# ymxlzgy/echoscene

Measured on AMD Instinct MI355X. Metric: denoising steps/sec (layout+SDF) for 32-node scene-graph, 64^3 SDF (3x16^3 latent), full step = one DDPM layout step + one DDIM shape step over all objects; `value` = the FUSED step (both loops as one hipGraph per step, the layout step on a parallel branch: what the K timed steps ran); `full_steps_p, higher is better.
Workload: dtype f16 MFMA operands / f32 accumulate (shape UNet); f32 (layout, GCN)

## Files before the change

echoscene_amd/csrc/es_vol.hip:

```cpp
#include "es_common.h"
#include <string>
#include <algorithm>
#include <cstdlib>
#include <initializer_list>
#include <utility>
#include <type_traits>

namespace {

__device__ __forceinline__ int f_swz(int row) { return (0x1320 >> (((row >> 2) & 3) * 4)) & 3; }

constexpr int GN_VT = 64;

__global__ __launch_bounds__(256) void k_gn_partial(const es_gn_args a, float* part, int vt) {
    __shared__ float ssum4[4][2048], ssq4[4][2048];
    float* ssum = ssum4[0];
    float* ssq = ssq4[0];
    const int o = blockIdx.y, tile = blockIdx.x, C = a.C1 + a.C2;
    const int v0 = tile * vt;
    const int nv = min(vt, a.V - v0);
    const int c4n = C >> 2;
    const int CX = 64;
    const int cx = threadIdx.x & (CX - 1), vy = threadIdx.x >> 6;
    for (int c4 = cx; c4 < c4n; c4 += CX) {
// ... 390 lines not shown
        const int w = (gy - p * Pw) < Pw ? (gy - p * Pw) : Pw;
        bx = rr / w;
        by = p * Pw + (rr - bx * w);
    } else {
        bx = t % gx;
        by = t / gx;
    }
}

__device__ __forceinline__ void* uniform_ptr(const void* p) {
    const unsigned long v = (unsigned long)p;
    const unsigned lo = (unsigned)__builtin_amdgcn_readfirstlane((int)(unsigned)v), hi = (unsigned)__builtin_amdgcn_readfirstlane((int)(unsigned)(v >> 32));
    return (void*)(((unsigned long)hi << 32) | lo);
}

template <int BM_, int NW_, bool ACTIVE = true, bool LOWREG = false, int EPI_ = -1, bool NOSYNC = false, bool STATS_ = false, bool FOLD_ = false>
__device__ __forceinline__ void conv_epilogue(const es_conv_args& a, const ConvGeom& g, f4 (&acc)[BM_ / (NW_ / 2) / 16][7],
                                              char* smem, long M, long m0, int n0, int wave, int lane, int S, int bz,
                                              int ncdhw) {
    constexpr int WROWS = BM_ / (NW_ / 2), MI = WROWS / 16;
    const bool geglu_epi = EPI_ < 0 ? a.epilogue == ES_EPI_GEGLU : EPI_ == ES_EPI_GEGLU;
    if constexpr (!ACTIVE) {
        __syncthreads();
        return;
    }
    const int wm = wave >> 1, wn = wave & 1, i16 = lane & 15, q = lane >> 4;
    const int V = g.D * g.H * g.W;
    if constexpr (!NOSYNC) __syncthreads();
    float* slab = (float*)smem + wave * (16 * 116);
    const bool vec_ok = !ncdhw && (a.N % 4 == 0) && (a.out_ld % 4 == 0) && (!a.rowvec || a.rowvec_ld % 4 == 0);
    float* part = S > 1 ? (float*)a.workspace + (long)bz * M * a.N : nullptr;
    if (geglu_epi) {
        const bool lo = i16 < 8;
        const int cw = i16 & 7;
#pragma unroll
        for (int j = 0; j < 7; ++j) {
            const float bj = a.bias[n0 + wn * 112 + j * 16 + i16];
#pragma unroll
            for (int i = 0; i < MI; ++i)
#pragma unroll
                for (int r = 0; r < 4; ++r) acc[i][j][r] += bj;
        }
        constexpr int HLD = 72;
        _Float16* hslab = (_Float16*)smem + wave * (16 * HLD);
        typedef unsigned int u4g __attribute__((ext_vector_type(4)));
        const int rr = q * 4 + (lo ? 0 : 2);
// ... 120 lines not shown
                }
                return;
            }
            f4 rbuf[2][8];
            write_slab(0);
            __builtin_amdgcn_sched_barrier(0);
            load_res_s(0, rbuf[0]);
            __builtin_amdgcn_sched_barrier(0);
#pragma unroll
            for (int i = 0; i < MI; ++i) {
                __builtin_amdgcn_s_waitcnt(0xc07f);
                __builtin_amdgcn_wave_barrier();
                if (i >= 1 && i + 1 < MI) load_res_s(i + 1, rbuf[(i + 1) & 1]);
                __builtin_amdgcn_sched_barrier(0);
                combine_s(i, rbuf[i & 1]);
                __builtin_amdgcn_sched_barrier(0);
                __builtin_amdgcn_wave_barrier();
                if (i + 1 < MI) write_slab(i + 1);
                __builtin_amdgcn_sched_barrier(0);
                if (i == 0 && MI > 1) load_res_s(1, rbuf[1]);
                __builtin_amdgcn_sched_barrier(0);
            }
            if constexpr (STATS_) {
                static_assert(WROWS == 64, "row groups of gn_stats_out are 64 rows");
                f4 os, oq;
#pragma unroll
                for (int e = 0; e < 4; ++e) { os[e] = __shfl(gs[e], lane + 28); oq[e] = __shfl(gq[e], lane + 28); }
                if (lane < 28 && n_ok && rows_left > 0) {
                    const unsigned nrg = (unsigned)((M + 63) >> 6);
                    const unsigned so = (unsigned)(mw0 >> 6) * (unsigned)a.N + (unsigned)n;
                    *(f4*)&a.gn_stats_out[so] = gs + os;
                    *(f4*)&a.gn_stats_out[so + nrg * (unsigned)a.N] = gq + oq;
                }
            }
        }
        return;
    }
#pragma unroll
    for (int i = 0; i < MI; ++i) {
        if (vec_ok) {
#pragma unroll
            for (int j = 0; j < 7; ++j)
#pragma unroll
                for (int r = 0; r < 4; ++r) slab[(q * 4 + r) * 116 + j * 16 + i16] = acc[i][j][r];
            __builtin_amdgcn_s_waitcnt(0xc07f);
            __builtin_amdgcn_wave_barrier();
            {
                typedef unsigned int u4e __attribute__((ext_vector_type(4)));
                typedef unsigned int u2e __attribute__((ext_vector_type(2)));
                constexpr unsigned OOBE = 0x80000000u;
                const long rb = m0 + wm * WROWS + i * 16;
                const int vshe = g.lw + g.lh + g.ld;
                float* const o32 = part ? part + rb * a.N : (a.out_f32 ? a.out_f32 + rb * a.out_ld : nullptr);
                const unsigned ldp = part ? (unsigned)a.N : (unsigned)a.out_ld, lde = (unsigned)a.out_ld;
                const bool ep = !part;
// ... 592 lines not shown
    conv_tile_of(a, bx, by, bz);
    const int S = gridDim.z;
    int ks_begin, ks_end;
    split_range(a.taps * (a.Cin >> 5), a.a2 ? (a.Cin2 >> 5) : 0, a.taps, bz, S, ks_begin, ks_end);
    conv_ws_tile<BM_, NC_, NP_, UP_, EPI_, STATS_, NS_>(a, g, ncdhw, smem, wave, lane, M, bx, by, ks_begin, ks_end, S, bz, stamp);
}

template <bool STATS_>
__global__ __launch_bounds__(768, 3) void k_conv_ws_fold(const es_conv_args a, const ConvGeom g) {
    extern __shared__ __attribute__((aligned(16))) char smem[];
    const int tid = threadIdx.x, lane = tid & 63;
    const int wave = __builtin_amdgcn_readfirstlane(tid >> 6);
    unsigned long long* stamp = nullptr;
#ifdef ES_STAMP
    stamp = g_stamp_buf ? g_stamp_buf + ((size_t)(blockIdx.x + gridDim.x * (blockIdx.y + gridDim.y * blockIdx.z)) * 12 + wave) * 8 : nullptr;
#endif
    ES_STAMP_AT(0);
    const long M = (long)g.O * g.D * g.H * g.W;
    int bx, by, bz;
    conv_tile_of(a, bx, by, bz);
    conv_ws_tile<256, 8, 4, true, ES_EPI_NONE, STATS_, 3, true>(a, g, 0, smem, wave, lane, M, bx, by, 0, 12 * (a.Cin >> 5), 1, 0, stamp);
}

typedef int i4v __attribute__((ext_vector_type(4)));
template <int DIR>
__device__ __forceinline__ h8 a3_shift(const h8 v, const bool zero_lane) {
    i4v x = __builtin_bit_cast(i4v, v);
#pragma unroll
    for (int e = 0; e < 4; ++e) {
        const int s = DIR < 0 ? __builtin_amdgcn_update_dpp(0, x[e], 0x111, 0xf, 0xf, true) : __builtin_amdgcn_update_dpp(0, x[e], 0x101, 0xf, 0xf, true);
        x[e] = zero_lane ? 0 : s;
    }
    return __builtin_bit_cast(h8, x);
}

template <bool STATS_>
__global__ __launch_bounds__(768, 3) void k_conv_ws3(const es_conv_args a, const ConvGeom g) {
    constexpr int BM_ = 256, NC_ = 8, NP_ = 4, NSB = 7, MI = 4;
    constexpr int A_BYTES = BM_ * BK * 2, B_BYTES = BNP * BK * 2, A_RING = NSB * B_BYTES;
    constexpr int NA = (BM_ / 16) / NP_, NB = (BNP / 16) / NP_;
    constexpr unsigned OOB = 0x80000000u;
    typedef __attribute__((address_space(3))) void* lds_ptr;
    extern __shared__ __attribute__((aligned(16))) char smem[];
    const int tid = threadIdx.x, lane = tid & 63;
    const int wave = __builtin_amdgcn_readfirstlane(tid >> 6);
    const long M = (long)g.O * g.D * g.H * g.W;
// ... 1277 lines not shown
    "ws_256_up_fold", "linear_ws", "linear_deep", "lean_256", "lean_128", "lean_64"
};
static_assert(sizeof(kConvKernelName) / sizeof(kConvKernelName[0]) == (size_t)ConvKernel::lean_64 + 1, "kConvKernelName: one name per ConvKernel value");
enum class ConvReduce { none, plain, gn_part };
struct ConvRoute {
    ConvGeom g;
    int ncdhw;
    long M;
    long omax;
    ConvKernel kernel;
    dim3 grid;
    size_t lds;
    int S;
    int ncb;
    bool upm, geglu;
    char unbuilt[96];
    bool epi_stats;
    bool stats;
    bool part_ok;
    ConvReduce reduce;
    int vt;
    bool stats_pass;
    int slabs;
};
}

constexpr int LDS256 = 3 * (256 * BK * 2 + BNP * BK * 2), LDS128 = 3 * (128 * BK * 2 + BNP * BK * 2), LDS64 = 3 * (64 * BK * 2 + BNP * BK * 2);
constexpr int LDSLIN = LDS256 + 8 * 16 * 116 * 4;
constexpr int LDSDEEP = 7 * (64 * BK * 2 + BNP * BK * 2);
constexpr int LDSWS3 = 9 * 16384;

static int conv_route(const es_conv_args* a, ConvRoute* r) {
    *r = ConvRoute{};
    ES_REQUIRE(a->Cin % 32 == 0 && a->Cin > 0, "es_conv_mfma_f16: Cin=%d must be a positive multiple of 32", a->Cin);
    ES_REQUIRE(a->taps == 27 || a->taps == 1, "es_conv_mfma_f16: taps=%d", a->taps);
    ES_REQUIRE(!a->a2 || (a->Cin2 % 32 == 0 && a->Cin2 > 0), "es_conv_mfma_f16: Cin2=%d", a->Cin2);
    ES_REQUIRE(a->out_f32 || a->out_f16, "es_conv_mfma_f16: no output");
    ES_REQUIRE(a->epilogue == ES_EPI_NONE || (a->epilogue == ES_EPI_GEGLU && a->N % 224 == 0 && a->out_f16 && !a->out_f32 && !a->res &&
                                              !a->rowvec && !a->a2 && a->bias && a->out_ld >= a->N / 2 && a->out_ld % 8 == 0 && a->splitk <= 1),
               "es_conv_mfma_f16: GEGLU epilogue needs N %% 224 == 0 (N=%d), bias, f16 output only, no split-K", a->N);
    ConvGeom& g = r->g;
    g.O = a->O; g.D = a->D; g.H = a->H; g.W = a->W;
    g.Hi = a->H; g.Wi = a->W;
    g.Di = a->D;
    if (a->mode == ES_CONV_DOWN_HW) { g.Hi = 2 * a->H; g.Wi = 2 * a->W; }
    ES_REQUIRE(a->mode >= ES_CONV_SAME && a->mode <= ES_CONV_DOWN_DHW_P01, "es_conv_mfma_f16: unknown mode %d", a->mode);
// ... 179 lines not shown
    } else if (st_bm) {
        const int np = vo("conv_st_np"), ns = vo("conv_st_ns");
        if (st_bm == 64 && np == 4 && ns == 3) r->kernel = ConvKernel::ws_64_4_4_3;
        else if (st_bm == 64 && np == 4 && ns == 6) r->kernel = ConvKernel::ws_64_4_4_6;
        else if (st_bm == 128 && np == 4 && ns == 3) r->kernel = ConvKernel::ws_128_4_4_3;
        else if (st_bm == 128 && np == 8 && ns == 3) r->kernel = ConvKernel::ws_128_4_8_3;
        else if (st_bm == 128 && np == 8 && ns == 5) r->kernel = ConvKernel::ws_128_4_8_5;
        else snprintf(r->unbuilt, sizeof(r->unbuilt), "conv_st_bm=%d conv_st_np=%d conv_st_ns=%d is not a built tile", st_bm, np, ns);
        r->grid = dim3((unsigned)((M + st_bm - 1) / st_bm), uy, S);
    } else if (deep) {
        S = 1;
        r->kernel = ConvKernel::linear_deep;
        r->grid = dim3((unsigned)((M + 63) / 64), uy, 1);
    } else if (route256) {
        r->grid = dim3((unsigned)((M + 255) / 256), uy, S);
        if (ncb > 1) {
            r->kernel = ConvKernel::linear_ws;
            r->grid = dim3(r->grid.x, (unsigned)(ntn / ncb), 1);
        } else if (ws && (!geglu || !upm)) {
            static const char* a3_env = getenv("ES_CONV_A3");
            const bool a3 = (a3_env ? atoi(a3_env) != 0 : ES_CONV_A3_DEFAULT) && a->taps == 27 && a->mode == ES_CONV_SAME && !a->a2 && a->W <= 16 && a->W >= 4;
            r->kernel = a3 ? ConvKernel::ws3 : ConvKernel::ws_256_8_4_3;
            if (r->kernel == ConvKernel::ws_256_8_4_3 && a->mode == ES_CONV_UP_HW && a->w2 && !a->a2 && S == 1 && a->O_hint == 0 &&
                a->H >= 2 && a->W >= 2 && ((long)a->D * g.Hi * g.Wi) % 256 == 0)
                r->kernel = ConvKernel::ws_256_up_fold;
        } else
            r->kernel = ConvKernel::lean_256;
    } else if ((wg128 >= 512 || S > 1) && !tiny_split) {
        r->kernel = ConvKernel::lean_128;
        r->grid = dim3((unsigned)((M + 127) / 128), uy, S);
    } else {
        r->kernel = ConvKernel::lean_64;
        r->grid = dim3((unsigned)((M + 63) / 64), uy, tiny_split ? S : 1);
    }
    r->S = S;
    if (S > 1) {
        r->reduce = a->gn_part_out && part_ok ? ConvReduce::gn_part : ConvReduce::plain;
        if (r->reduce == ConvReduce::gn_part) r->vt = gn_voxel_tile(Oh, a->D * a->H * a->W);
    }
    return 0;
}

template <int BM_, int NC_, int NP_, int NS_>
static int launch_ws(const es_conv_args* a, const ConvRoute& r, hipStream_t st) {
    constexpr int LDS = NS_ * (BM_ * BK * 2 + BNP * BK * 2);
    constexpr bool CAN_STATS = BM_ / (NC_ / 2) == 64;
    static_assert(LDS <= 160 * 1024, "ring exceeds the CU's LDS");
    static const LdsLimits lim{{(const void*)k_conv_ws<BM_, NC_, NP_, false, ES_EPI_NONE, false, NS_>, LDS},
// ... 33 lines not shown

template <int BM_, int NW_>
static void launch_lean(const es_conv_args* a, const ConvRoute& r, hipStream_t st) {
    constexpr int LDS = 3 * (BM_ * BK * 2 + BNP * BK * 2);
    if (r.upm) hipLaunchKernelGGL((k_conv_lean<BM_, NW_, true>), r.grid, dim3(64 * NW_), LDS, st, *a, r.g, r.ncdhw);
    else hipLaunchKernelGGL((k_conv_lean<BM_, NW_>), r.grid, dim3(64 * NW_), LDS, st, *a, r.g, r.ncdhw);
}

static void launch_rowgroup_stats(const es_conv_args* a, long rows, hipStream_t st) {
    const long n4 = ((rows + 63) / 64) * (a->N / 4);
    const int blocks = (int)((n4 + 255) / 256 < 8192 ? (n4 + 255) / 256 : 8192);
    hipLaunchKernelGGL(k_rowgroup_stats, dim3(blocks), dim3(256), 0, st, (const float*)a->out_f32, rows, a->N, a->out_ld, a->gn_stats_out);
}

static int conv_launch(const es_conv_args* a, const ConvRoute& r, hipStream_t st) {
    static const LdsLimits lim{{(const void*)k_conv_small_n_tiled, 160 * 1024},
                               {(const void*)k_conv_n16, N16_A_BYTES + N16_B_BYTES},
                               {(const void*)k_conv_lean<256, 8>, LDS256}, {(const void*)k_conv_lean<256, 8, true>, LDS256},
                               {(const void*)k_conv_lean<128, 4>, LDS128}, {(const void*)k_conv_lean<128, 4, true>, LDS128},
                               {(const void*)k_conv_lean<64, 4>, LDS64}, {(const void*)k_conv_lean<64, 4, true>, LDS64},
                               {(const void*)k_linear_deep, LDSDEEP},
                               {(const void*)k_linear_ws<ES_EPI_NONE>, LDSLIN}, {(const void*)k_linear_ws<ES_EPI_GEGLU>, LDSLIN},
                               {(const void*)k_conv_ws3<false>, LDSWS3}, {(const void*)k_conv_ws3<true>, LDSWS3},
                               {(const void*)k_conv_ws_fold<false>, LDS256}, {(const void*)k_conv_ws_fold<true>, LDS256}};
    ES_REQUIRE(lim.err == hipSuccess, "es_conv_mfma_f16: hipFuncSetAttribute failed: %s", hipGetErrorString(lim.err));
    ES_REQUIRE(r.kernel != ConvKernel::none, "es_conv_mfma_f16: %s", r.omax ? "a chunked route is launched chunk by chunk" : r.unbuilt);
    int rc = 0;
    switch (r.kernel) {
    case ConvKernel::none: break;
    case ConvKernel::small_n:
    case ConvKernel::small_n_tiled:
        ES_REQUIRE(a->mode == ES_CONV_SAME && !a->a2 && !a->res && !a->rowvec && !a->out_f16 && !a->gn_stats_out,
                   "es_conv_mfma_f16: the N<=4, Cin<=64 direct kernel takes SAME mode, fp32 output, no fusions");
        if (r.kernel == ConvKernel::small_n_tiled) hipLaunchKernelGGL(k_conv_small_n_tiled, r.grid, dim3(256), r.lds, st, *a, r.g, r.ncdhw);
        else hipLaunchKernelGGL(k_conv_small_n, r.grid, dim3(256), r.lds, st, *a, r.g, r.ncdhw);
        break;
    case ConvKernel::n16: hipLaunchKernelGGL(k_conv_n16, r.grid, dim3(256), N16_A_BYTES + N16_B_BYTES, st, *a, r.g); break;
    case ConvKernel::kw_4_1: rc = launch_kw<4, 1>(a, r, st); break;
    case ConvKernel::kw_2_2: rc = launch_kw<2, 2>(a, r, st); break;
    case ConvKernel::ws_256_8_4_3: rc = launch_ws<256, 8, 4, 3>(a, r, st); break;
    case ConvKernel::ws_64_4_4_3: rc = launch_ws<64, 4, 4, 3>(a, r, st); break;
    case ConvKernel::ws_64_4_4_6: rc = launch_ws<64, 4, 4, 6>(a, r, st); break;
    case ConvKernel::ws_128_4_4_3: rc = launch_ws<128, 4, 4, 3>(a, r, st); break;
    case ConvKernel::ws_128_4_8_3: rc = launch_ws<128, 4, 8, 3>(a, r, st); break;
    case ConvKernel::ws_128_4_8_5: rc = launch_ws<128, 4, 8, 5>(a, r, st); break;
    case ConvKernel::ws3:
        if (r.stats) hipLaunchKernelGGL((k_conv_ws3<true>), r.grid, dim3(768), LDSWS3, st, *a, r.g);
        else hipLaunchKernelGGL((k_conv_ws3<false>), r.grid, dim3(768), LDSWS3, st, *a, r.g);
        break;
    case ConvKernel::ws_256_up_fold:
        if (r.stats) hipLaunchKernelGGL((k_conv_ws_fold<true>), r.grid, dim3(768), LDS256, st, *a, r.g);
        else hipLaunchKernelGGL((k_conv_ws_fold<false>), r.grid, dim3(768), LDS256, st, *a, r.g);
        break;
    case ConvKernel::linear_ws:
        if (r.geglu) hipLaunchKernelGGL((k_linear_ws<ES_EPI_GEGLU>), r.grid, dim3(768), LDSLIN, st, *a, r.g, r.ncb);
        else hipLaunchKernelGGL((k_linear_ws<ES_EPI_NONE>), r.grid, dim3(768), LDSLIN, st, *a, r.g, r.ncb);
        break;
    case ConvKernel::linear_deep: hipLaunchKernelGGL(k_linear_deep, r.grid, dim3(256), LDSDEEP, st, *a, r.g); break;
    case ConvKernel::lean_256: launch_lean<256, 8>(a, r, st); break;
    case ConvKernel::lean_128: launch_lean<128, 4>(a, r, st); break;
    case ConvKernel::lean_64: launch_lean<64, 4>(a, r, st); break;
    }
    if (rc) return rc;
    const int V = a->D * a->H * a->W;
    if (r.reduce == ConvReduce::gn_part)
        hipLaunchKernelGGL(k_conv_splitk_reduce_gn, dim3((V + r.vt - 1) / r.vt, a->O), dim3(256), 0, st, *a, r.M, V, r.S, r.vt);
    else if (r.reduce == ConvReduce::plain) {
        const long n4 = r.M * (a->N / 4);
        const int blocks = (int)((n4 + 255) / 256 < 4096 ? (n4 + 255) / 256 : 4096);
        hipLaunchKernelGGL(k_conv_splitk_reduce, dim3(blocks), dim3(256), 0, st, *a, r.M, V, r.S);
    }
    if (r.stats_pass) {
        ES_REQUIRE(a->out_f32, "es_conv_mfma_f16: this launch's route forms gn_stats_out by a pass over the fp32 output: out_f32 must be given "
                               "(es_conv_emits_gn_stats() == 0)");
// ... 37 lines not shown
    return 0;
}

extern "C" int es_conv_emits_gn_stats(const es_conv_args* a) {
    ConvRoute r;
    return conv_route(a, &r) == 0 ? (int)r.epi_stats : -1;
}

extern "C" int es_conv_emits_gn_part(const es_conv_args* a) {
    ConvRoute r;
    return conv_route(a, &r) == 0 ? (int)r.part_ok : -1;
}

extern "C" int es_conv_split_of(const es_conv_args* a) {
    ConvRoute r;
    return conv_route(a, &r) == 0 ? r.slabs : -1;
}

extern "C" int es_conv_kernel_of(const es_conv_args* a, char* name_out, int cap) {
    ConvRoute r;
    if (conv_route(a, &r) != 0) return -1;
    if (name_out && cap > 0) snprintf(name_out, (size_t)cap, "%s", r.omax ? "chunked" : kConvKernelName[(int)r.kernel]);
    return r.S > 1 ? r.S : 1;
}

extern "C" int es_groupnorm_vol(const es_gn_args* a, es_stream stream) {
    const int C = a->C1 + a->C2;
    ES_REQUIRE(C % a->groups == 0 && C <= 2048 && a->groups <= 64, "es_groupnorm_vol: C=%d groups=%d", C, a->groups);
    ES_REQUIRE(a->C1 % 8 == 0 && a->C2 % 8 == 0, "es_groupnorm_vol: channel counts must be multiples of 8 (%d,%d)", a->C1, a->C2);
    ES_REQUIRE(a->stats != nullptr, "es_groupnorm_vol: stats scratch missing");
    const long Oh = a->O_hint < 0 ? -(long)a->O_hint : (long)(a->O_hint > a->O ? a->O_hint : a->O);
    const int vt = gn_voxel_tile(Oh, a->V);
    const int ntiles = (a->V + vt - 1) / vt;
    float* part = a->stats;
    const bool from_rg = a->stats1 && (!a->x2 || a->stats2) && a->V % 64 == 0 && (a->x1_is_f16 || vo("gn_rg") != 0);
    ES_REQUIRE(!a->x1_is_f16 || (from_rg && !a->x2 && !a->raw_f16),
               "es_groupnorm_vol: an f16 source needs the producer's row-group sums (stats1), one source, no raw copy");
    ES_REQUIRE(!a->part_in || (!from_rg && !a->x2), "es_groupnorm_vol: part_in needs one source and no row-group sums");
    if (a->part_in) part = (float*)a->part_in;
    else if (!from_rg) hipLaunchKernelGGL(k_gn_partial, dim3(ntiles, a->O), dim3(256), 0, (hipStream_t)stream, *a, part, vt);
    int vpb = 32;
    while (vpb > 8 && (long)a->O * ((a->V + vpb - 1) / vpb) < 512) vpb >>= 1;
    while (vpb < 1024 && (long)a->O * ((a->V + vpb - 1) / vpb) > 16384) vpb <<= 1;
    const float* fin = nullptr;
    if (from_rg) {
        hipLaunchKernelGGL(k_gn_finalize_rg, dim3(a->groups, a->O), dim3(256), 0, (hipStream_t)stream, *a, part);
// ... 87 lines not shown
```

echoscene_amd/hip.py:

```python
import ctypes as C
import os

HERE = os.path.dirname(os.path.abspath(__file__))
LIB_PATH = os.path.join(HERE, 'libechoscene_hip%s.so' % os.environ.get('ES_LIB_TAG', ''))

c_f32p = C.c_void_p
c_i32p = C.c_void_p

SEG_DIRECT, SEG_GATHER, SEG_CSRMEAN, SEG_CSRSUM, SEG_CSRWAVG = 0, 1, 2, 3, 4
PRO_NONE, PRO_SILU, PRO_GN, PRO_GN_SILU, PRO_LN, PRO_GEGLU, PRO_LN_ATTN = 0, 1, 2, 3, 4, 5, 6
ACT_NONE, ACT_RELU, ACT_SILU, ACT_GEGLU, ACT_SIGMOID = 0, 1, 2, 3, 4
CONV_SAME, CONV_DOWN_HW, CONV_UP_HW, CONV_UP_DHW, CONV_DOWN_DHW = 0, 1, 2, 3, 4
CONV_DOWN_DHW_P01 = 5
EPI_NONE, EPI_GEGLU = 0, 1
(OP_LINEAR, OP_DDPM, OP_DDIM, OP_COPY, OP_CONV, OP_GN, OP_LN, OP_ATTN, OP_GEGLU, OP_TO_CL, OP_STEM) = range(1, 12)
OP_VQ = 12
OP_FORK, OP_JOIN, OP_ROWSEL = 13, 14, 15
OP_CONV_F32, OP_ATTN_F32 = 16, 17
OP_DDIM_BLEND, OP_CONV_C1 = 18, 19
OP_DDPM_KEEP = 21


class Seg(C.Structure):
    _fields_ = [('ptr', C.c_void_p), ('idx', C.c_void_p), ('ent_row', C.c_void_p), ('ent_off', C.c_void_p),
# ... 144 lines not shown
    'es_linear_rows_slices': (C.c_int, [C.POINTER(LinearArgs), C.POINTER(C.c_int)]),
    'es_linear_rows_takes_ln_attn': (C.c_int, [C.POINTER(LinearArgs)]),
    'es_linear_rows_auto_slices': (C.c_int, [C.c_int, C.c_int, C.c_int]),
    'es_row_select': (C.c_int, [C.POINTER(RowSelArgs), C.c_void_p]),
    'es_ddpm_update': (C.c_int, [C.POINTER(UpdateArgs), C.c_void_p]),
    'es_ddim_update': (C.c_int, [C.POINTER(UpdateArgs), C.c_void_p]),
    'es_ddim_blend': (C.c_int, [C.POINTER(BlendArgs), C.c_void_p]),
    'es_conv_c1_f32': (C.c_int, [C.POINTER(ConvC1Args), C.c_void_p]),
    'es_ddpm_update_keep': (C.c_int, [C.POINTER(DdpmKeepArgs), C.c_void_p]),
    'es_ddim_rows_update': (C.c_int, [C.POINTER(DdpmKeepArgs), C.c_void_p]),
    'es_plms_update': (C.c_int, [C.POINTER(PlmsArgs), C.c_void_p]),
    'es_plms_first_a': (C.c_int, [C.POINTER(PlmsArgs), C.c_void_p]),
    'es_plms_first_b': (C.c_int, [C.POINTER(PlmsArgs), C.c_void_p]),
    'es_box_prescale': (C.c_int, [C.c_void_p, C.c_int, C.c_int, C.c_void_p, C.c_void_p, C.c_void_p, C.c_int, C.c_void_p, C.c_int,
                                  C.c_void_p]),
    'es_box_postprocess': (C.c_int, [C.c_void_p, C.c_int, C.c_void_p, C.c_void_p, C.c_void_p, C.c_int, C.c_float,
                                     C.c_void_p]),
    'es_box_descale': (C.c_int, [C.c_void_p, C.c_int, C.c_int, C.c_void_p, C.c_int, C.c_void_p]),
    'es_conv_mfma_f16': (C.c_int, [C.POINTER(ConvArgs), C.c_void_p]),
    'es_conv_emits_gn_stats': (C.c_int, [C.POINTER(ConvArgs)]),
    'es_conv_emits_gn_part': (C.c_int, [C.POINTER(ConvArgs)]),
    'es_conv_split_of': (C.c_int, [C.POINTER(ConvArgs)]),
    'es_conv_kernel_of': (C.c_int, [C.POINTER(ConvArgs), C.c_char_p, C.c_int]),
    'es_split_f16x3': (C.c_int, [C.c_void_p, C.c_long, C.c_int, C.c_void_p, C.c_void_p]),
    'es_pack_conv_f16_size': (C.c_size_t, [C.c_int, C.c_int, C.c_int]),
    'es_pack_conv_f16': (C.c_int, [C.c_void_p, C.c_int, C.c_int, C.c_int, C.c_void_p]),
    'es_pack_conv_f16_dev': (C.c_int, [C.c_void_p, C.c_int, C.c_int, C.c_int, C.c_void_p, C.c_void_p]),
    'es_pack_conv_rows_f16': (C.c_int, [C.c_void_p, C.c_int, C.c_int, C.c_int, C.c_void_p]),
    'es_pack_conv_up_fold_f16_size': (C.c_size_t, [C.c_int, C.c_int]),
    'es_pack_conv_up_fold_f16': (C.c_int, [C.c_void_p, C.c_int, C.c_int, C.c_void_p]),
    'es_pack_conv_up_fold_f16_dev': (C.c_int, [C.c_void_p, C.c_int, C.c_int, C.c_void_p, C.c_void_p]),
    'es_groupnorm_vol': (C.c_int, [C.POINTER(GNArgs), C.c_void_p]),
    'es_layernorm_tokens': (C.c_int, [C.POINTER(LNArgs), C.c_void_p]),
    'es_attention_f16': (C.c_int, [C.POINTER(AttnArgs), C.c_void_p]),
    'es_geglu_f16': (C.c_int, [C.POINTER(GegluArgs), C.c_void_p]),
    'es_latent_to_cl_f16': (C.c_int, [C.c_void_p, C.c_int, C.c_int, C.c_int, C.c_int, C.c_void_p, C.c_void_p]),
    'es_latent_to_cl_f32': (C.c_int, [C.c_void_p, C.c_int, C.c_int, C.c_int, C.c_int, C.c_void_p, C.c_void_p]),
    'es_pack_conv_f32_size': (C.c_size_t, [C.c_int, C.c_int, C.c_int]),
    'es_pack_conv_f32': (C.c_int, [C.c_void_p, C.c_int, C.c_int, C.c_int, C.c_void_p]),
    'es_conv_f32': (C.c_int, [C.POINTER(ConvArgs), C.c_void_p]),
    'es_attention_f32': (C.c_int, [C.POINTER(AttnArgs), C.c_void_p]),
    'es_shape_stem': (C.c_int, [C.POINTER(StemArgs), C.c_void_p]),
    'es_vq_lookup': (C.c_int, [C.POINTER(VQArgs), C.c_void_p]),
    'es_init': (C.c_int, []),
    'es_chamfer_forward': (C.c_int, [C.c_void_p, C.c_void_p, C.c_int, C.c_int, C.c_int, C.c_void_p, C.c_void_p, C.c_void_p,
                                     C.c_void_p, C.c_void_p]),
# ... 62 lines not shown
```

echoscene_amd/plan_vol.py:

```python
import ctypes as C
import os
import torch

from . import hip
from .hip import ConvArgs, GNArgs, LNArgs, AttnArgs, GegluArgs, ToClArgs, StemArgs, BlendArgs, ConvC1Args, Op
from .plan import (Builder, PackedLinear, GCNWeights, View, seg, emit_gcn, own, mm64)


VOL_FOLD_FFO = True
VOL_GN_F16 = True
VOL_GN_PART_FUSED = True
VOL_GN_RG_ANY = False


def _gn_rg():
    buf = C.create_string_buffer(512)
    hip.lib().es_vol_options(buf, 512)
    opts = dict(kv.split('=') for kv in buf.value.decode().strip(';').split(';'))
    return int(opts.get('gn_rg', '1')) != 0


def up_fold_weights(W):
    W = W.detach().double().cpu()
    assert W.dim() == 5 and tuple(W.shape[2:]) == (3, 3, 3)
# ... 167 lines not shown
            elif kind == 'up':
                if precision == 'fp16' and not self.concat:
                    d['conv'] = PackedConv(sd[name + '.conv.weight'], sd[name + '.conv.bias'], device, up_fold=True)
                else:
                    d['conv'] = PC(name + '.conv.weight', name + '.conv.bias')
            self.items[name] = d
        self.emb_all = PackedLinear(torch.cat(emb_w, 0), torch.cat(emb_b, 0), device)
        self.cav_all = None if self.concat else PackedLinear(torch.cat(ca_v, 0), torch.cat(ca_b, 0), device)
        self.out_gn = (dv('out.0.weight'), dv('out.0.bias'))
        self.out_conv = PC('out.2.weight', 'out.2.bias')
        self.in_ch, self.out_ch = net.in_channels, net.out_channels


class VolBuilderMixin:

    def _push(self, kind, field, a):
        op = Op()
        op.kind, op.lane = kind, 0
        setattr(op.u, field, a)
        self.ops.append(op)
        return len(self.ops) - 1

    def conv(self, a_f16, pc, O, dims, mode=hip.CONV_SAME, bias=None, rowvec=None, res=None, out_f32=None,
             out_f16=None, skip=None, ncdhw=False, splitk=None, epilogue=0, out_ld=None):
        D, H, W = dims
        if getattr(self, 'fp32x', False) and a_f16.dtype == torch.float32:
            assert isinstance(pc, PackedConvX3) and not epilogue
            a3 = self.split3(a_f16, pc.cin_part)
            if skip is not None:
                skip = (self.split3(skip[0], skip[1].cin_part), skip[1])
            out = out_f32 if out_f32 is not None else out_f16
            assert out is not None and out.dtype == torch.float32 and (out_f32 is None or out_f16 is None)
            return self.conv(a3, pc, O, dims, mode=mode, bias=bias, rowvec=rowvec, res=res, out_f32=out, skip=skip, ncdhw=ncdhw,
                             splitk=splitk, out_ld=out_ld)
        if getattr(self, 'fp32', False) and not getattr(self, 'fp32x', False):
            return self._conv32(a_f16, pc, O, dims, mode, bias, rowvec, res, out_f32, out_f16, skip, ncdhw, out_ld)
        a = ConvArgs()
        a.a, a.w = a_f16.data_ptr(), pc.w.data_ptr()
        a.O, a.D, a.H, a.W = O, D, H, W
        a.Cin, a.N, a.taps, a.mode = pc.Cin, pc.N, pc.taps, mode
        if skip is not None:
            a.a2, a.w2, a.Cin2 = skip[0].data_ptr(), skip[1].w.data_ptr(), skip[1].Cin
            self.weight_bytes += skip[1].weight_bytes
            self.flops += 2 * O * D * H * W * skip[1].Cin * pc.N
        bt = pc.b if bias is None else bias
        a.bias = bt.data_ptr() if bt is not None else None
        if rowvec is not None:
            a.rowvec, a.rowvec_ld = rowvec.ptr, rowvec.ld
        a.res = res.data_ptr() if res is not None else None
        a.out_f32 = out_f32.data_ptr() if out_f32 is not None else None
        a.out_f16 = out_f16.data_ptr() if out_f16 is not None else None
        a.out_ld = -1 if ncdhw else (pc.N if out_ld is None else out_ld)
        a.epilogue = epilogue
        a.O_hint = int(getattr(self, 'o_hint', 0) or 0)
        M = O * D * H * W
        Mh = (-a.O_hint if a.O_hint < 0 else max(a.O_hint, O)) * D * H * W
        if not ncdhw and Mh * pc.N <= 8192 * 5376 and pc.N % 4 == 0 and not epilogue:
            a.splitk = -1 if splitk is None else splitk
            a.workspace = 1
            S = hip.lib().es_conv_split_of(C.byref(a))
            if S < 0:
                raise RuntimeError('es_conv_split_of: ' + hip.lib().es_last_error().decode())
            need = max(S, splitk or 0, 1) * M * pc.N
            if getattr(self, '_ws', None) is None or self._ws.numel() < need:
                self._ws = self.buf(need, scratch=True)
                for op in self.ops:
                    if op.kind == hip.OP_CONV and op.u.conv.workspace:
                        op.u.conv.workspace = self._ws.data_ptr()
            a.workspace = self._ws.data_ptr()
        self.keep += [pc, bt, skip]
        self.weight_bytes += pc.weight_bytes
        self.flops += 2 * O * D * H * W * pc.cin_true * pc.taps * pc.N
        idx = self._push(hip.OP_CONV, 'conv', a)
        if out_f32 is not None and not ncdhw and not epilogue and (out_ld is None or out_ld == pc.N):
            if not hasattr(self, '_conv_of'):
                self._conv_of = {}
            self._conv_of[out_f32.data_ptr()] = (idx, M, pc.N)
        return idx

    def split3(self, x32, C):
# ... 433 lines not shown
                    gl = sbuf(M, 8 * Cc)
                    b.conv(l3, d['ff1'], O, dm, out_f32=gl)
                    b.geglu(gl, M, 4 * Cc, gg)
                o = sbuf(M, Cc)
                if 'ffo' in d:
                    state['last_op'] = b.conv(gg, d['ffo'], O, dm, bias=d['ffo_bias'], skip=(t2 if b.fp32 else t2h, d['po']), res=xin, out_f32=o)
                else:
                    t3 = sbuf(M, Cc, dtype=f16)
                    b.conv(gg, d['ff2'], O, dm, res=t2, out_f16=t3)
                    state['last_op'] = b.conv(t3, d['proj_out'], O, dm, res=xin, out_f32=o)
                b.tags[name + '.transformer_blocks.0:in'] = View(t0)
                b.tags[name + '.transformer_blocks.0:attn2'] = View(t2)
                state.update(h=o, h16=None)
            elif kind == 'down':
                a16 = need_f16()
                nd = (dm[0] // 2, dm[1] // 2, dm[2] // 2) if w.concat else (dm[0], dm[1] // 2, dm[2] // 2)
                o = sbuf(O * V_(nd), state['C'])
                state['last_op'] = b.conv(a16, d['conv'], O, nd, mode=hip.CONV_DOWN_DHW if w.concat else hip.CONV_DOWN_HW, out_f32=o)
                state.update(h=o, dims=nd, h16=None)
            elif kind == 'up':
                a16 = need_f16()
                nd = (dm[0] * 2, dm[1] * 2, dm[2] * 2) if w.concat else (dm[0], dm[1] * 2, dm[2] * 2)
                o = sbuf(O * V_(nd), state['C'])
                state['last_op'] = b.conv(a16, d['conv'], O, nd, mode=hip.CONV_UP_DHW if w.concat else hip.CONV_UP_HW, out_f32=o)
                wf = getattr(d['conv'], 'w_fold', None)
                if (wf is not None and getattr(b, 'up_fold', False) and not w.concat and not b.fp32
                        and not int(getattr(b, 'o_hint', 0) or 0)):
                    b.ops[state['last_op']].u.conv.w2 = wf.data_ptr()
                    b.keep.append(wf)
                state.update(h=o, dims=nd, h16=None)
            b.tags[name] = View(state['h'])

    inp, mid, out = w.topo
    hs = []
    for i, blk in enumerate(inp):
        run_block(f'input_blocks.{i}', blk)
        hs.append((state['h'], state['C']))
    run_block('middle_block', mid)
    for i, blk in enumerate(out):
        run_block(f'output_blocks.{i}', blk, skip=hs.pop())
    join_side()
    dm = state['dims']
    yo = sbuf(O * V_(dm), state['C'], dtype=f16)
    b.groupnorm(state['h'], state['C'], None, 0, O, V_(dm), w.out_gn[0], w.out_gn[1], 1e-5, True, yo)
    b.conv(yo, w.out_conv, O, dm, out_f32=eps_out, ncdhw=True)
    return objbuf


for _n in ('_push', 'conv', '_conv32', 'split3', 'conv_gn_intermediate', '_rowgroup_producer', '_rowgroup_stats', 'groupnorm', 'layernorm', 'attention', 'geglu', 'to_cl', 'stem', 'conv_c1', 'blend', 'plms'):
    setattr(Builder, _n, getattr(VolBuilderMixin, _n))


# ... 215 lines not shown
```

include/echoscene_hip.h:

```cpp
#ifndef ECHOSCENE_HIP_H
#define ECHOSCENE_HIP_H

#include <stddef.h>
#include <stdint.h>

#ifdef __cplusplus
extern "C" {
#endif

typedef void* es_stream;
typedef struct es_plan es_plan;

#define ES_ABI_VERSION 10
int es_abi_version(void);
const char* es_last_error(void);
int es_device_info(char* name_out, int name_cap, int* cu_count);

enum { ES_SEG_DIRECT = 0, ES_SEG_GATHER = 1, ES_SEG_CSRMEAN = 2, ES_SEG_CSRSUM = 3, ES_SEG_CSRWAVG = 4 };
enum { ES_PRO_NONE = 0, ES_PRO_SILU = 1, ES_PRO_GN = 2, ES_PRO_GN_SILU = 3, ES_PRO_LN = 4, ES_PRO_GEGLU = 5, ES_PRO_LN_ATTN = 6 };
enum { ES_ACT_NONE = 0, ES_ACT_RELU = 1, ES_ACT_SILU = 2, ES_ACT_GEGLU = 3, ES_ACT_SIGMOID = 4 };

typedef struct es_seg {
    const float* ptr;
    const int32_t* idx;
// ... 142 lines not shown
    int32_t mode;
    const void* a2; const void* w2; int32_t Cin2;
    const float* bias;
    const float* rowvec;
    int32_t rowvec_ld;
    const float* res;
    float* out_f32;
    void* out_f16;
    void* workspace;
    int32_t splitk;
    int32_t out_ld;
    int32_t O_hint;
    int32_t epilogue;
    float* gn_stats_out;
    float* gn_part_out;
    int32_t gn_part_groups;
} es_conv_args;
enum { ES_EPI_NONE = 0, ES_EPI_GEGLU = 1 };
int es_conv_mfma_f16(const es_conv_args* args, es_stream stream);
int es_conv_emits_gn_stats(const es_conv_args* args);
int es_conv_emits_gn_part(const es_conv_args* args);
int es_conv_split_of(const es_conv_args* args);
int es_conv_kernel_of(const es_conv_args* args, char* name_out, int cap);
int es_split_f16x3(const float* x, long M, int C, void* out, es_stream stream);
size_t es_pack_conv_f16_size(int N, int Cin, int taps);
int es_pack_conv_f16(const float* h_w, int N, int Cin, int taps, uint16_t* h_out);
int es_pack_conv_f16_dev(const float* d_w, int N, int Cin, int taps, uint16_t* d_out, es_stream stream);
int es_pack_conv_rows_f16(const float* h_w, int N, int Cin, int taps, uint16_t* h_out);
size_t es_pack_conv_up_fold_f16_size(int N, int Cin);
int es_pack_conv_up_fold_f16(const float* h_w, int N, int Cin, uint16_t* h_out);
int es_pack_conv_up_fold_f16_dev(const float* d_w, int N, int Cin, uint16_t* d_out, es_stream stream);

typedef struct es_gn_args {
    const float* x1; int32_t C1;
    const float* x2; int32_t C2;
    int32_t O, V;
    int32_t groups; float eps;
    const float* gamma; const float* beta;
    int32_t silu;
    float* stats;
    void* y_f16;
    void* raw_f16;
    int32_t O_hint;
    const float* stats1;
    const float* stats2;
    int32_t x1_is_f16;
// ... 139 lines not shown
```

Before: 56.52.

## Balance fold-upsample conv waves with a 256+128 row tile split kernel

Adds a balanced variant of the up-fold conv kernel. When the 256-row tile grid would leave the last wave of workgroups underfilled, each workgroup runs one 256-row tile and then a 128-row tile, which evens out the tail. The GN stats epilogue is extended to 32-row wave groups, exchanging partial sums through LDS so the 64-row stat groups stay intact. The Python planner now passes the fold weights to the conv builder before routing, so folded convs skip the split-K workspace path. This adds extra barriers and more LDS traffic in the stats epilogue.

```diff
diff --git a/echoscene_amd/csrc/es_vol.hip b/echoscene_amd/csrc/es_vol.hip
--- a/echoscene_amd/csrc/es_vol.hip
+++ b/echoscene_amd/csrc/es_vol.hip
@@ -436,6 +436,7 @@
     const bool geglu_epi = EPI_ < 0 ? a.epilogue == ES_EPI_GEGLU : EPI_ == ES_EPI_GEGLU;
     if constexpr (!ACTIVE) {
         __syncthreads();
+        if constexpr (STATS_ && WROWS == 32) __syncthreads();
         return;
     }
     const int wm = wave >> 1, wn = wave & 1, i16 = lane & 15, q = lane >> 4;
@@ -602,15 +603,28 @@
                 __builtin_amdgcn_sched_barrier(0);
             }
             if constexpr (STATS_) {
-                static_assert(WROWS == 64, "row groups of gn_stats_out are 64 rows");
+                static_assert(WROWS == 64 || (WROWS == 32 && FOLD_), "row groups of gn_stats_out are 64 rows");
                 f4 os, oq;
 #pragma unroll
                 for (int e = 0; e < 4; ++e) { os[e] = __shfl(gs[e], lane + 28); oq[e] = __shfl(gq[e], lane + 28); }
+                if constexpr (WROWS == 64) {
                 if (lane < 28 && n_ok && rows_left > 0) {
                     const unsigned nrg = (unsigned)((M + 63) >> 6);
                     const unsigned so = (unsigned)(mw0 >> 6) * (unsigned)a.N + (unsigned)n;
                     *(f4*)&a.gn_stats_out[so] = gs + os;
                     *(f4*)&a.gn_stats_out[so + nrg * (unsigned)a.N] = gq + oq;
+                }
+                } else {
+                    f4* const xch = (f4*)(smem + NW_ * (16 * 116) * 4) + (wave * 28 + (lane < 28 ? lane : 0)) * 2;
+                    if (!(wm & 1) && lane < 28) { xch[0] = gs + os; xch[1] = gq + oq; }
+                    __syncthreads();
+                    if ((wm & 1) && lane < 28 && n_ok && rows_left > 0) {
+                        const f4* const lo = xch - 2 * 28 * 2;
+                        const unsigned nrg = (unsigned)((M + 63) >> 6);
+                        const unsigned so = (unsigned)(mw0 >> 6) * (unsigned)a.N + (unsigned)n;
+                        *(f4*)&a.gn_stats_out[so] = lo[0] + (gs + os);
+                        *(f4*)&a.gn_stats_out[so + nrg * (unsigned)a.N] = lo[1] + (gq + oq);
+                    }
                 }
             }
         }
@@ -1249,6 +1263,20 @@
     conv_ws_tile<256, 8, 4, true, ES_EPI_NONE, STATS_, 3, true>(a, g, 0, smem, wave, lane, M, bx, by, 0, 12 * (a.Cin >> 5), 1, 0, stamp);
 }
 
+template <bool STATS_>
+__global__ __launch_bounds__(768, 3) void k_conv_ws_fold_bal(const es_conv_args a, const ConvGeom g) {
+    extern __shared__ __attribute__((aligned(16))) char smem[];
+    const int tid = threadIdx.x, lane = tid & 63;
+    const int wave = __builtin_amdgcn_readfirstlane(tid >> 6);
+    const long M = (long)g.O * g.D * g.H * g.W;
+    int bx, by, bz;
+    conv_tile_of(a, bx, by, bz);
+    const int nks = 12 * (a.Cin >> 5);
+    conv_ws_tile<256, 8, 4, true, ES_EPI_NONE, STATS_, 3, true>(a, g, 0, smem, wave, lane, M, bx, by, 0, nks, 1, 0, nullptr);
+    __syncthreads();
+    conv_ws_tile<128, 8, 4, true, ES_EPI_NONE, STATS_, 3, true>(a, g, 0, smem, wave, lane, M, 2 * bx + by, 2, 0, nks, 1, 0, nullptr);
+}
+
 typedef int i4v __attribute__((ext_vector_type(4)));
 template <int DIR>
 __device__ __forceinline__ h8 a3_shift(const h8 v, const bool zero_lane) {
@@ -2572,6 +2600,7 @@
     int vt;
     bool stats_pass;
     int slabs;
+    bool fold_bal;
 };
 }
 
@@ -2797,8 +2826,14 @@
             const bool a3 = (a3_env ? atoi(a3_env) != 0 : ES_CONV_A3_DEFAULT) && a->taps == 27 && a->mode == ES_CONV_SAME && !a->a2 && a->W <= 16 && a->W >= 4;
             r->kernel = a3 ? ConvKernel::ws3 : ConvKernel::ws_256_8_4_3;
             if (r->kernel == ConvKernel::ws_256_8_4_3 && a->mode == ES_CONV_UP_HW && a->w2 && !a->a2 && S == 1 && a->O_hint == 0 &&
-                a->H >= 2 && a->W >= 2 && ((long)a->D * g.Hi * g.Wi) % 256 == 0)
+                a->H >= 2 && a->W >= 2 && ((long)a->D * g.Hi * g.Wi) % 256 == 0) {
                 r->kernel = ConvKernel::ws_256_up_fold;
+                const long rounds = (wg256 + 255) / 256;
+                if (ntn == 3 && !a->workspace && M % 256 == 0 && (double)wg256 / (double)(rounds * 256) < 0.8) {
+                    r->fold_bal = true;
+                    r->grid = dim3(r->grid.x, 2, 1);
+                }
+            }
         } else
             r->kernel = ConvKernel::lean_256;
     } else if ((wg128 >= 512 || S > 1) && !tiny_split) {
@@ -2878,7 +2913,8 @@
                                {(const void*)k_linear_deep, LDSDEEP},
                                {(const void*)k_linear_ws<ES_EPI_NONE>, LDSLIN}, {(const void*)k_linear_ws<ES_EPI_GEGLU>, LDSLIN},
                                {(const void*)k_conv_ws3<false>, LDSWS3}, {(const void*)k_conv_ws3<true>, LDSWS3},
-                               {(const void*)k_conv_ws_fold<false>, LDS256}, {(const void*)k_conv_ws_fold<true>, LDS256}};
+                               {(const void*)k_conv_ws_fold<false>, LDS256}, {(const void*)k_conv_ws_fold<true>, LDS256},
+                               {(const void*)k_conv_ws_fold_bal<false>, LDS256}, {(const void*)k_conv_ws_fold_bal<true>, LDS256}};
     ES_REQUIRE(lim.err == hipSuccess, "es_conv_mfma_f16: hipFuncSetAttribute failed: %s", hipGetErrorString(lim.err));
     ES_REQUIRE(r.kernel != ConvKernel::none, "es_conv_mfma_f16: %s", r.omax ? "a chunked route is launched chunk by chunk" : r.unbuilt);
     int rc = 0;
@@ -2905,7 +2941,10 @@
         else hipLaunchKernelGGL((k_conv_ws3<false>), r.grid, dim3(768), LDSWS3, st, *a, r.g);
         break;
     case ConvKernel::ws_256_up_fold:
-        if (r.stats) hipLaunchKernelGGL((k_conv_ws_fold<true>), r.grid, dim3(768), LDS256, st, *a, r.g);
+        if (r.fold_bal) {
+            if (r.stats) hipLaunchKernelGGL((k_conv_ws_fold_bal<true>), r.grid, dim3(768), LDS256, st, *a, r.g);
+            else hipLaunchKernelGGL((k_conv_ws_fold_bal<false>), r.grid, dim3(768), LDS256, st, *a, r.g);
+        } else if (r.stats) hipLaunchKernelGGL((k_conv_ws_fold<true>), r.grid, dim3(768), LDS256, st, *a, r.g);
         else hipLaunchKernelGGL((k_conv_ws_fold<false>), r.grid, dim3(768), LDS256, st, *a, r.g);
         break;
     case ConvKernel::linear_ws:
@@ -2989,6 +3028,11 @@
     if (conv_route(a, &r) != 0) return -1;
     if (name_out && cap > 0) snprintf(name_out, (size_t)cap, "%s", r.omax ? "chunked" : kConvKernelName[(int)r.kernel]);
     return r.S > 1 ? r.S : 1;
+}
+
+extern "C" int es_conv_fold_balanced(const es_conv_args* a) {
+    ConvRoute r;
+    return conv_route(a, &r) == 0 ? (int)r.fold_bal : -1;
 }
 
 extern "C" int es_groupnorm_vol(const es_gn_args* a, es_stream stream) {
diff --git a/echoscene_amd/hip.py b/echoscene_amd/hip.py
--- a/echoscene_amd/hip.py
+++ b/echoscene_amd/hip.py
@@ -190,6 +190,7 @@
     'es_conv_emits_gn_part': (C.c_int, [C.POINTER(ConvArgs)]),
     'es_conv_split_of': (C.c_int, [C.POINTER(ConvArgs)]),
     'es_conv_kernel_of': (C.c_int, [C.POINTER(ConvArgs), C.c_char_p, C.c_int]),
+    'es_conv_fold_balanced': (C.c_int, [C.POINTER(ConvArgs)]),
     'es_split_f16x3': (C.c_int, [C.c_void_p, C.c_long, C.c_int, C.c_void_p, C.c_void_p]),
     'es_pack_conv_f16_size': (C.c_size_t, [C.c_int, C.c_int, C.c_int]),
     'es_pack_conv_f16': (C.c_int, [C.c_void_p, C.c_int, C.c_int, C.c_int, C.c_void_p]),
diff --git a/echoscene_amd/plan_vol.py b/echoscene_amd/plan_vol.py
--- a/echoscene_amd/plan_vol.py
+++ b/echoscene_amd/plan_vol.py
@@ -213,8 +213,9 @@
         return len(self.ops) - 1
 
     def conv(self, a_f16, pc, O, dims, mode=hip.CONV_SAME, bias=None, rowvec=None, res=None, out_f32=None,
-             out_f16=None, skip=None, ncdhw=False, splitk=None, epilogue=0, out_ld=None):
+             out_f16=None, skip=None, ncdhw=False, splitk=None, epilogue=0, out_ld=None, w_fold=None):
         D, H, W = dims
+        assert w_fold is None or (skip is None and mode == hip.CONV_UP_HW)
         if getattr(self, 'fp32x', False) and a_f16.dtype == torch.float32:
             assert isinstance(pc, PackedConvX3) and not epilogue
             a3 = self.split3(a_f16, pc.cin_part)
@@ -246,7 +247,15 @@
         a.O_hint = int(getattr(self, 'o_hint', 0) or 0)
         M = O * D * H * W
         Mh = (-a.O_hint if a.O_hint < 0 else max(a.O_hint, O)) * D * H * W
-        if not ncdhw and Mh * pc.N <= 8192 * 5376 and pc.N % 4 == 0 and not epilogue:
+        folded = False
+        if w_fold is not None:
+            a.w2 = w_fold.data_ptr()
+            self.keep.append(w_fold)
+            name = C.create_string_buffer(32)
+            if hip.lib().es_conv_kernel_of(C.byref(a), name, 32) < 0:
+                raise RuntimeError('es_conv_kernel_of: ' + hip.lib().es_last_error().decode())
+            folded = name.value == b'ws_256_up_fold'
+        if not folded and not ncdhw and Mh * pc.N <= 8192 * 5376 and pc.N % 4 == 0 and not epilogue:
             a.splitk = -1 if splitk is None else splitk
             a.workspace = 1
             S = hip.lib().es_conv_split_of(C.byref(a))
@@ -726,12 +735,11 @@
                 a16 = need_f16()
                 nd = (dm[0] * 2, dm[1] * 2, dm[2] * 2) if w.concat else (dm[0], dm[1] * 2, dm[2] * 2)
                 o = sbuf(O * V_(nd), state['C'])
-                state['last_op'] = b.conv(a16, d['conv'], O, nd, mode=hip.CONV_UP_DHW if w.concat else hip.CONV_UP_HW, out_f32=o)
                 wf = getattr(d['conv'], 'w_fold', None)
-                if (wf is not None and getattr(b, 'up_fold', False) and not w.concat and not b.fp32
+                if not (wf is not None and getattr(b, 'up_fold', False) and not w.concat and not b.fp32
                         and not int(getattr(b, 'o_hint', 0) or 0)):
-                    b.ops[state['last_op']].u.conv.w2 = wf.data_ptr()
-                    b.keep.append(wf)
+                    wf = None
+                state['last_op'] = b.conv(a16, d['conv'], O, nd, mode=hip.CONV_UP_DHW if w.concat else hip.CONV_UP_HW, out_f32=o, w_fold=wf)
                 state.update(h=o, dims=nd, h16=None)
             b.tags[name] = View(state['h'])
 
diff --git a/include/echoscene_hip.h b/include/echoscene_hip.h
--- a/include/echoscene_hip.h
+++ b/include/echoscene_hip.h
@@ -188,6 +188,7 @@
 int es_conv_emits_gn_part(const es_conv_args* args);
 int es_conv_split_of(const es_conv_args* args);
 int es_conv_kernel_of(const es_conv_args* args, char* name_out, int cap);
+int es_conv_fold_balanced(const es_conv_args* args);
 int es_split_f16x3(const float* x, long M, int C, void* out, es_stream stream);
 size_t es_pack_conv_f16_size(int N, int Cin, int taps);
 int es_pack_conv_f16(const float* h_w, int N, int Cin, int taps, uint16_t* h_out);
```

New measurement: 57.40, median of 6. +1.5%, better.
